# jamie8johnson/cqs

Measured on AMD Instinct MI355X. Metric: queries/sec @k=20 (brute-force cosine scan + top-k, 768-d fp32), higher is better.
Workload: dtype f32; 1 GPU; BASELINE configs[1]: 1000000 x 768 fp32 unit vectors, 1 query per step, brute-force cosine top-20; mode=single, rows_per_gpu=1000000, total_rows=1000000, dim=768, k=20, parallelism=single GPU, ranks_seen=1

## Files before the change

cqs_amd/csrc/index.hip:

```cpp
#include <hip/hip_runtime.h>

#include <algorithm>
#include <atomic>
#include <cmath>
#include <cerrno>
#include <chrono>
#include <cstdio>
#include <cstdlib>
#include <cstring>
#include <mutex>
#include <new>
#include <string>
#include <thread>
#include <vector>

#include <fcntl.h>
#include <libgen.h>
#include <sys/stat.h>
#include <unistd.h>

#include "abi_guard.h"
#include "roctx.h"
#include "index_internal.h"
#include "persist_util.h"
// ... 1 lines not shown
#include "scan_i8.h"

using cqs::kMaxK;
using cqs::kRowsPerBlock;

namespace cqs_idx {

uint64_t pad_rows(uint64_t n) { return (n + kRowsPerBlock - 1) / kRowsPerBlock * kRowsPerBlock; }

int32_t fail(cqs_hip_index* idx, int32_t code, const char* what, hipError_t e) {
    char buf[512];
    if (e != hipSuccess)
        snprintf(buf, sizeof buf, "%s: %s (%s)", what, hipGetErrorString(e), hipGetErrorName(e));
    else
        snprintf(buf, sizeof buf, "%s", what);
    if (idx) {
        idx->last_error = buf;
        if (code == CQS_HIP_ERR_DEVICE) idx->poisoned.store(true, std::memory_order_release);
    }
    return code;
}

void free_scratch(cqs_hip_index* x) {
    hipFree(x->d_q); hipFree(x->d_scores); hipFree(x->d_gmax); hipFree(x->d_work); hipFree(x->d_gaux);
    x->d_work = nullptr; x->d_gaux = nullptr;
    hipFree(x->d_out_keys); hipFree(x->d_out_counts);
    hipHostFree(x->h_q); hipHostFree(x->h_out_keys); hipHostFree(x->h_out_counts);
    x->d_q = x->d_scores = nullptr; x->d_gmax = nullptr;
    x->d_out_keys = nullptr; x->d_out_counts = nullptr;
    x->h_q = nullptr; x->h_out_keys = nullptr; x->h_out_counts = nullptr;
    x->h_out_keys_dev = nullptr; x->h_out_counts_dev = nullptr;
    x->q_cap = 0; x->k_cap = 0; x->scr_n_pad = 0;
}

int32_t ensure_scratch(cqs_hip_index* x, uint32_t b, uint32_t k) {
    const uint64_t n_pad = pad_rows(x->n);
    if (b <= x->q_cap && k <= x->k_cap && n_pad == x->scr_n_pad) return CQS_HIP_OK;
    HIP_TRY(x, hipDeviceSynchronize());
    uint32_t qc = x->q_cap > b ? x->q_cap : b;
    uint32_t kc = x->k_cap > k ? x->k_cap : k;
    free_scratch(x);
    HIP_TRY(x, hipMalloc(&x->d_q, ((size_t)qc + 256) * x->dim * sizeof(float)));
    HIP_TRY(x, hipMalloc(&x->d_scores, (size_t)qc * n_pad * sizeof(float)));
    HIP_TRY(x, hipMalloc(&x->d_work, cqs::kWorkWords * sizeof(uint32_t)));
    HIP_TRY(x, hipMemset(x->d_work, 0, cqs::kWorkWords * sizeof(uint32_t)));
    HIP_TRY(x, hipMalloc(&x->d_gmax, (size_t)qc * (n_pad / cqs::kTaskRowsSmall) * sizeof(float)));
    HIP_TRY(x, hipMalloc(&x->d_gaux, (size_t)(qc < kGauxQueries ? qc : kGauxQueries) * (n_pad / cqs::kTaskRowsSmall) * sizeof(uint64_t)));
    HIP_TRY(x, hipMalloc(&x->d_out_keys, (size_t)qc * kc * sizeof(uint64_t)));
    HIP_TRY(x, hipMalloc(&x->d_out_counts, (size_t)qc * sizeof(uint32_t)));
    HIP_TRY(x, hipHostMalloc(&x->h_q, (size_t)qc * x->dim * sizeof(float), hipHostMallocDefault));
    HIP_TRY(x, hipHostMalloc(&x->h_out_keys, (size_t)qc * kc * sizeof(uint64_t), hipHostMallocDefault));
    HIP_TRY(x, hipHostMalloc(&x->h_out_counts, (size_t)qc * sizeof(uint32_t), hipHostMallocDefault));
    if (hipHostGetDevicePointer((void**)&x->h_out_keys_dev, x->h_out_keys, 0) != hipSuccess ||
        hipHostGetDevicePointer((void**)&x->h_out_counts_dev, x->h_out_counts, 0) != hipSuccess) {
        (void)hipGetLastError();
        x->h_out_keys_dev = nullptr; x->h_out_counts_dev = nullptr;
    }
    x->q_cap = qc; x->k_cap = kc; x->scr_n_pad = n_pad;
    return CQS_HIP_OK;
}

uint32_t max_query_block(const cqs_hip_index* x) {
    const uint64_t budget = 16ull << 30;
    const uint64_t per_q = pad_rows(x->n) * sizeof(float);
    uint64_t q = per_q ? budget / per_q : 1024;
    if (q < 1) q = 1;
    if (q > 1024) q = 1024;
    return (uint32_t)q;
}

// ... 1043 lines not shown
```

cqs_amd/csrc/index_internal.h:

```cpp
#pragma once
#include <hip/hip_runtime.h>

#include <atomic>
#include <chrono>
#include <condition_variable>
#include <deque>
#include <mutex>
#include <string>
#include <vector>

#include "../../include/cqs_hip.h"
#include "scan_kernels.h"

namespace cqs_sharded { struct ShardSet; }
namespace cqs_idx { struct Shadow; }
namespace cqs_mmr { struct Scratch; }

struct cqs_combine_req {
    const float* q;
    uint32_t k, mode;
    float thr;
    uint64_t* out_rows;
    float* out_scores;
    uint32_t* out_count;
// ... 3 lines not shown
};

struct cqs_hip_index {
    int device = 0;
    uint64_t n = 0;
    uint64_t cap_rows = 0;
    uint32_t dim = 0;
    uint32_t metric = 0;
    uint64_t row_base = 0;
    bool borrow = false;
    float* d_rows = nullptr;
    hipStream_t stream = nullptr;

    uint32_t q_cap = 0;
    uint64_t scr_n_pad = 0;
    uint32_t k_cap = 0;
    float* d_q = nullptr;
    float* d_scores = nullptr;
    uint32_t* d_work = nullptr;
    unsigned long long* d_dbg = nullptr;
    uint32_t n_cu = 256;
    float* d_gmax = nullptr;
    uint64_t* d_gaux = nullptr;
    uint64_t* d_out_keys = nullptr;
    uint32_t* d_out_counts = nullptr;
    uint32_t* d_keep = nullptr;
    uint64_t keep_words_cap = 0;
    uint32_t* d_keep_tab = nullptr;
    uint32_t* h_keep_tab = nullptr;
    uint64_t keep_tab_stride = 0;
    float* h_q = nullptr;
    uint64_t* h_out_keys = nullptr;
    uint32_t* h_out_counts = nullptr;
    uint64_t* h_out_keys_dev = nullptr;
    uint32_t* h_out_counts_dev = nullptr;

    hipEvent_t done = nullptr;
    hipStream_t done_stream = nullptr;
    bool done_valid = false;

    bool timing = false;
    std::vector<hipEvent_t> ev;
    size_t ev_used = 0;

    cqs_sharded::ShardSet* sh = nullptr;

// ... 121 lines not shown
```

cqs_amd/csrc/index_shadow.hip:

```cpp
#include <cstdlib>
#include <cstring>
#include <new>

#include "abi_guard.h"
#include "index_internal.h"
#include "scan_bf16.h"
#include "scan_i8.h"

namespace cqs_idx {

constexpr uint64_t kShadowAutoBytes = 1ull << 30;
constexpr uint64_t kShadowFreeMinBytes = 4ull << 30;
constexpr double kShadowFreeFrac = 0.10;
constexpr uint32_t kStatWords = 10, kStatCounts = 3, kStatI8 = 5, kStatI8Counts = 8;

struct Shadow {
    uint16_t* d_bf16 = nullptr;
    uint64_t cap = 0;
    int8_t* d_i8 = nullptr;
    float* d_i8_scale = nullptr;
    double r8 = 0.0, norm8 = 0.0;
    double r = 0.0;
    double norm = 0.0;
    unsigned long long* d_stats = nullptr;
// ... 235 lines not shown
bool shadow_takes(const cqs_hip_index* x, uint32_t b, uint32_t k, bool gemv_only) {
    return x->shadow && b <= cqs::kShadowMaxQ && (gemv_only || !cqs::use_mfma(b, x->dim)) && cqs::shadow_kprime(k) >= k;
}

bool shadow_uses_i8(const cqs_hip_index* x, uint32_t b, uint32_t k) {
    return x->shadow && x->shadow->d_i8 && b <= cqs::kI8MaxQ && cqs::i8_k_ok(k);
}

int32_t shadow_pass(cqs_hip_index* x, const float* d_q, uint32_t nb, uint32_t k, const uint32_t* d_keep, uint32_t mode,
                    float threshold, uint64_t* out_keys, uint32_t* out_counts, hipStream_t st, const uint32_t** device_gate,
                    const KeepTab* tab) {
    const Shadow* s = x->shadow;
    uint32_t* const cert = device_gate || !s->h_cert_dev ? s->d_cert : s->h_cert_dev;
    if (device_gate) *device_gate = cert;
    if (device_gate) HIP_TRY(x, order_after_last(x, st));
    const bool i8 = shadow_uses_i8(x, nb, k);
    const uint32_t kp = i8 ? cqs::i8_kprime(k) : cqs::shadow_kprime(k);
    const double r_max = i8 ? s->r8 : s->r, norm_max = i8 ? s->norm8 : s->norm;
    const bool bound_first = mode == CQS_HIP_MODE_PIPELINE;
    if (bound_first) {
        if (i8) HIP_TRY(x, cqs::launch_i8_bound(d_q, nb, x->dim, r_max, norm_max, s->d_bq, st));
        else HIP_TRY(x, cqs::launch_shadow_bound(d_q, nb, x->dim, r_max, norm_max, s->d_bq, st));
    }
    const cqs::ScanArgs a = scan_args(x, d_q, nb, kp + 1u, d_keep, mode, threshold, i8 ? sizeof(int8_t) : sizeof(uint16_t), true, nullptr, nullptr, tab);
    const ShadowRows rows{i8 ? nullptr : s->d_bf16, i8 ? s->d_i8 : nullptr, s->d_i8_scale, s->d_bq};
    const int32_t rc = scan_select(x, a, st, &rows, nullptr, nullptr);
    if (rc == CQS_HIP_OK)
        HIP_TRY(x, cqs::launch_rescore_certify(a, (uint32_t)x->row_base, k, kp, bound_first ? 0u : (i8 ? 2u : 1u), r_max, norm_max,
                                               s->d_bq, s->d_tickets, s->d_ekeys, out_keys, out_counts, cert,
                                               device_gate ? s->d_stats + kStatCounts : nullptr,
                                               device_gate && i8 ? s->d_stats + kStatI8Counts : nullptr, st));
    return rc;
}

hipError_t shadow_verdicts(cqs_hip_index* x, uint32_t nb, const uint32_t** h_cert) {
    const Shadow* s = x->shadow;
    *h_cert = s->h_cert;
    return s->h_cert_dev ? hipSuccess : hipMemcpyAsync(s->h_cert, s->d_cert, (size_t)nb * sizeof(uint32_t), hipMemcpyDeviceToHost, x->stream);
}

}

using namespace cqs_idx;

extern "C" {

int32_t cqs_hip_index_set_bf16_scan(cqs_hip_index* x, int32_t enable) CQS_ABI_TRY {
// ... 148 lines not shown
        if ((rc = stage_keep(x, keep_bitset, (x->n + 31) / 32)) != CQS_HIP_OK) return rc;
        d_keep = x->d_keep;
    }
    hipStream_t st = x->stream;
    HIP_TRY(x, hipMemcpyAsync(x->d_q, queries, (size_t)b * x->dim * sizeof(float), hipMemcpyHostToDevice, st));
    if (i8) HIP_TRY(x, cqs::launch_i8_bound(x->d_q, b, x->dim, s->r8, s->norm8, s->d_bq, st));
    else HIP_TRY(x, cqs::launch_shadow_bound(x->d_q, b, x->dim, s->r, s->norm, s->d_bq, st));
    if (copy == 0u) {
        const cqs::ScanArgs a = scan_args(x, x->d_q, b, k, d_keep, mode, threshold, sizeof(float), false, x->d_dbg, nullptr);
        HIP_TRY(x, cqs::launch_scan(a, st));
    } else {
        const cqs::ScanArgs a = scan_args(x, x->d_q, b, k_scan, d_keep, mode, threshold, i8 ? sizeof(int8_t) : sizeof(uint16_t), true, nullptr, nullptr);
        if (i8) HIP_TRY(x, cqs::launch_scan_i8(a, s->d_i8, s->d_i8_scale, s->d_bq, st));
        else HIP_TRY(x, cqs::launch_scan_bf16(a, s->d_bf16, s->d_bq, st));
    }
    HIP_TRY(x, hipMemsetAsync(x->d_work, 0, cqs::kWorkWords * sizeof(uint32_t), st));
    const size_t row_b = (size_t)x->n * sizeof(float);
    HIP_TRY(x, hipMemcpy2DAsync(out_scores, row_b, x->d_scores, (size_t)pad_rows(x->n) * sizeof(float), row_b, b, hipMemcpyDeviceToHost, st));
    HIP_TRY(x, hipMemcpyAsync(out_bq, s->d_bq, (size_t)b * sizeof(float), hipMemcpyDeviceToHost, st));
    HIP_TRY(x, hipStreamSynchronize(st));
    return CQS_HIP_OK;
} CQS_ABI_CATCH(x)

}
```

cqs_amd/csrc/scan_bf16.hip:

```cpp
#include "scan_bf16.h"
#include "scan_i8.h"
#include "launch_util.h"
#include "rank_sort.h"
#include "scan_gemv_device.h"
#include "select_device.h"

namespace cqs {

static_assert(kShadowKMax == kMaxK, "shadow k' policy and the select agree on max k");

typedef __bf16 bf2 __attribute__((ext_vector_type(2)));

__device__ __forceinline__ float bf_lo(uint32_t w) { return __uint_as_float(w << 16); }
__device__ __forceinline__ float bf_hi(uint32_t w) { return __uint_as_float(w & 0xFFFF0000u); }
__device__ __forceinline__ float key_score(uint64_t key) {
    const uint32_t ok = (uint32_t)(key >> 32);
    return __uint_as_float((ok & 0x80000000u) ? (ok ^ 0x80000000u) : ~ok);
}

__global__ __launch_bounds__(256) void shadow_build_kernel(const float* __restrict__ rows, uint16_t* __restrict__ shadow,
                                                           uint64_t row0, uint64_t n_rows, uint32_t dim, double gamma,
                                                           unsigned long long* __restrict__ stats) {
    const int lane = threadIdx.x & 63;
    const uint64_t waves = (uint64_t)gridDim.x * (blockDim.x >> 6);
// ... 288 lines not shown
}

hipError_t launch_scan_bf16(const ScanArgs& a, const uint16_t* shadow, const float* bq, hipStream_t st) {
    if (a.b == 0 || a.n == 0) return hipSuccess;
    if (a.b > kShadowMaxQ || a.dim % 8u != 0u || a.dim > kShadowMaxDim) return hipErrorInvalidValue;
    if (a.keep_tab && !keep_tab_ok(a)) return hipErrorInvalidValue;
    switch ((a.dim + 511u) / 512u) {
        case 1: return a.keep_tab ? launch_bf16_groups<1, true>(a, shadow, bq, st) : launch_bf16_groups<1, false>(a, shadow, bq, st);
        case 2: return a.keep_tab ? launch_bf16_groups<2, true>(a, shadow, bq, st) : launch_bf16_groups<2, false>(a, shadow, bq, st);
        case 3: return a.keep_tab ? launch_bf16_groups<3, true>(a, shadow, bq, st) : launch_bf16_groups<3, false>(a, shadow, bq, st);
        case 4: return a.keep_tab ? launch_bf16_groups<4, true>(a, shadow, bq, st) : launch_bf16_groups<4, false>(a, shadow, bq, st);
        default: return hipErrorInvalidValue;
    }
}

struct TailParams {
    const float* rows;
    const float* q;
    uint32_t dim, k, kprime, mode, row_base;
    float thr;
    const float* scores;
    const float* gmax;
    const uint64_t* gaux;
    uint32_t n_pad;
    TaskTiers tiers;
    uint32_t bins;
    uint32_t* work;
    uint64_t* ekeys;
    float* bq;
    uint32_t* tickets;
    uint32_t bound;
    double r_max, norm_max;
    uint64_t* out_keys;
    uint32_t* out_counts;
    uint32_t* cert;
    unsigned long long* counters;
    unsigned long long* counters2;
};

constexpr uint32_t kTailWaves = 16;

template <int NCH>
__global__ __launch_bounds__(1024) void rescore_certify_kernel(const TailParams p) {
    __shared__ uint64_t s_keys[kShadowKMax];
    __shared__ uint64_t s_sorted[kShadowKMax];
    __shared__ __attribute__((aligned(16))) uint32_t s_ok[kShadowKMax + 4];
    __shared__ uint32_t s_cnt, s_flag, s_last;
    const uint32_t lane = threadIdx.x & 63u;
    const uint32_t qi = blockIdx.y;
    const uint32_t wave = (uint32_t)__builtin_amdgcn_readfirstlane((int)(blockIdx.x * kTailWaves + (threadIdx.x >> 6)));
    const uint32_t n_waves = gridDim.x * kTailWaves;
    const uint32_t dim = p.dim;
    const float* qp = p.q + (size_t)qi * dim;
    if (threadIdx.x == 0) s_cnt = 0u;
    if (qi == 0u && blockIdx.x == 0u)
        for (uint32_t i = threadIdx.x; i < kWorkWords; i += 1024u) p.work[i] = 0u;

    const uint32_t n_tasks = p.tiers.total();
    uint32_t found;
    const uint64_t* akeys = select_body(p.scores + (size_t)qi * p.n_pad, p.gmax + (size_t)qi * n_tasks,
                                        p.gaux ? p.gaux + (size_t)qi * n_tasks : nullptr, p.n_pad, p.tiers, p.kprime + 1u,
                                        p.row_base, p.bins, nullptr, found);
    const uint32_t ac = found < p.kprime + 1u ? found : p.kprime + 1u;
    const uint32_t nc = ac < p.kprime ? ac : p.kprime;
    const uint64_t key_next = ac > p.kprime ? akeys[p.kprime] : 0ull;

    for (uint32_t slot = wave; slot <= nc; slot += n_waves) {
        if (slot == 0u) {
            if (p.bound != 0u) {
                const float v = p.bound == 2u ? wave_i8_bound(qp, dim, p.r_max, p.norm_max, lane)
                                              : wave_shadow_bound(qp, dim, p.r_max, p.norm_max, lane);
                if (lane == 0u)
                    __hip_atomic_store((uint32_t*)p.bq + qi, __float_as_uint(v), __ATOMIC_RELAXED, __HIP_MEMORY_SCOPE_AGENT);
            }
            continue;
        }
        const uint32_t i = slot - 1u;
        const uint64_t key = akeys[i];
        const uint32_t grow = 0xFFFFFFFFu - (uint32_t)key;
        const float* rp = p.rows + (size_t)(grow - p.row_base) * dim;
        f4 x[NCH], qv[NCH];
#pragma unroll
        for (int c = 0; c < NCH; ++c) {
            const uint32_t idx = (uint32_t)c * 256u + lane * 4u;
            const bool in = idx < dim;
// ... 54 lines not shown
                if (p.mode == 1u) t = t < 0.f ? 0.f : (t > 1.f ? 1.f : t);
                ok = t < key_score(s_sorted[k - 1u]);
            }
        }
        p.cert[qi] = ok ? 1u : 0u;
        if (p.counters) atomicAdd(&p.counters[ok ? 0 : 1], 1ull);
        if (p.counters2) atomicAdd(&p.counters2[ok ? 0 : 1], 1ull);
    }
}

#ifndef CQS_TAIL_MAX_BLOCKS_PER_CU
#define CQS_TAIL_MAX_BLOCKS_PER_CU 1u
#endif

hipError_t launch_rescore_certify(const ScanArgs& a, uint32_t row_base, uint32_t k, uint32_t kprime, uint32_t bound,
                                  double r_max, double norm_max, float* bq, uint32_t* tickets, uint64_t* ekeys,
                                  uint64_t* out_keys, uint32_t* out_counts, uint32_t* cert, unsigned long long* counters,
                                  unsigned long long* counters2, hipStream_t st) {
    const uint32_t b = a.b, dim = a.dim;
    if (b == 0) return hipSuccess;
    if (b > kShadowMaxQ || k == 0 || kprime < k || kprime >= kShadowKMax || a.k != kprime + 1u || dim % 8u != 0u ||
        dim > kShadowMaxDim || bound > 2u)
        return hipErrorInvalidValue;
    const TailParams tp{a.rows, a.q, dim, k, kprime, a.mode, row_base, a.threshold, a.scores, a.gmax, a.gaux, a.n_pad, a.tiers,
                        a.range_bins ? 2u : (a.linear_bins ? 1u : 0u), a.work, ekeys, bq, tickets, bound, r_max, norm_max,
                        out_keys, out_counts, cert, counters, counters2};
    const uint32_t want = (kprime + 1u + kTailWaves - 1u) / kTailWaves;
    uint32_t cap = a.n_cu * CQS_TAIL_MAX_BLOCKS_PER_CU / b;
    if (cap < 1u) cap = 1u;
    const dim3 grid(want < cap ? want : cap, b), block(64u * kTailWaves);
    switch ((dim + 255u) / 256u) {
        case 1: hipLaunchKernelGGL(rescore_certify_kernel<1>, grid, block, 0, st, tp); break;
        case 2: hipLaunchKernelGGL(rescore_certify_kernel<2>, grid, block, 0, st, tp); break;
        case 3: hipLaunchKernelGGL(rescore_certify_kernel<3>, grid, block, 0, st, tp); break;
        case 4: hipLaunchKernelGGL(rescore_certify_kernel<4>, grid, block, 0, st, tp); break;
        case 5: hipLaunchKernelGGL(rescore_certify_kernel<5>, grid, block, 0, st, tp); break;
        case 6: hipLaunchKernelGGL(rescore_certify_kernel<6>, grid, block, 0, st, tp); break;
        case 7: hipLaunchKernelGGL(rescore_certify_kernel<7>, grid, block, 0, st, tp); break;
        case 8: hipLaunchKernelGGL(rescore_certify_kernel<8>, grid, block, 0, st, tp); break;
        default: return hipErrorInvalidValue;
    }
    return hipGetLastError();
}

}
```

cqs_amd/csrc/scan_i8.hip:

```cpp
#include "scan_i8.h"
#include "launch_util.h"
#include "scan_gemv_device.h"

namespace cqs {

template <int I>
__device__ __forceinline__ float code_f32(uint32_t w) { return (float)(int)(int8_t)(w >> (8 * I)); }

constexpr int kI8BuildVecs = (int)(kShadowMaxDim / 256u);

__global__ __launch_bounds__(256) void i8_build_kernel(const float* __restrict__ rows, int8_t* __restrict__ codes,
                                                       float* __restrict__ scales, uint64_t row0, uint64_t n_rows,
                                                       uint32_t dim, double gamma, unsigned long long* __restrict__ stats) {
    const uint32_t lane = threadIdx.x & 63u;
    const uint64_t waves = (uint64_t)gridDim.x * (blockDim.x >> 6);
    for (uint64_t r = (uint64_t)blockIdx.x * (blockDim.x >> 6) + (threadIdx.x >> 6); r < n_rows; r += waves) {
        const float* xp = rows + (row0 + r) * dim;
        int8_t* op = codes + (row0 + r) * dim;
        f4 v[kI8BuildVecs];
        float m = 0.f;
        bool fin = true;
#pragma unroll
        for (int j = 0; j < kI8BuildVecs; ++j) {
            const uint32_t i = (uint32_t)j * 256u + lane * 4u;
// ... 48 lines not shown
hipError_t launch_i8_build(const float* rows, int8_t* codes, float* scales, uint64_t row0, uint64_t n_rows, uint32_t dim,
                           double gamma, unsigned long long* stats, hipStream_t st) {
    if (n_rows == 0) return hipSuccess;
    if (!i8_dim_ok(dim)) return hipErrorInvalidValue;
    const uint64_t blocks = (n_rows + 3u) / 4u;
    hipLaunchKernelGGL(i8_build_kernel, dim3((uint32_t)(blocks < 8192u ? blocks : 8192u)), dim3(256), 0, st, rows, codes,
                       scales, row0, n_rows, dim, gamma, stats);
    return hipGetLastError();
}

__global__ __launch_bounds__(64) void i8_bound_kernel(const float* __restrict__ q, uint32_t dim, double r_max,
                                                      double norm_max, float* __restrict__ bq) {
    const uint32_t lane = threadIdx.x;
    const float v = wave_i8_bound(q + (size_t)blockIdx.x * dim, dim, r_max, norm_max, lane);
    if (lane == 0) bq[blockIdx.x] = v;
}

hipError_t launch_i8_bound(const float* q, uint32_t b, uint32_t dim, double r_max, double norm_max, float* bq, hipStream_t st) {
    if (b == 0) return hipSuccess;
    if (b > kShadowMaxQ) return hipErrorInvalidValue;
    hipLaunchKernelGGL(i8_bound_kernel, dim3(b), dim3(64), 0, st, q, dim, r_max, norm_max, bq);
    return hipGetLastError();
}

struct I8ScanParams {
    const int8_t* rows;
    const float* scales;
    uint32_t n, n_pad, dim;
    const float* q;
    float* scores;
    const uint32_t* keep;
    uint32_t mode;
    float thr;
    uint32_t nq;
    TaskTiers tiers;
    uint32_t n_tasks;
    float* gmax;
    uint64_t* gaux;
    const float* bq;
    uint32_t keep_stride;
    uint8_t slot[kMaxGemvQ];
};

template <int NCH, int BQ, int RI, bool NT, bool FULL, bool PQ>
__global__ __launch_bounds__(256) void scan_i8_kernel(const I8ScanParams p) {
    constexpr int NV = RI * BQ;
    constexpr int LPV = 64 / NV;
    const int lane = threadIdx.x & 63;
    const uint32_t n = p.n, dim = p.dim;

    uint32_t coff[NCH];
    f4 qv[BQ][NCH][4];
#pragma unroll
    for (int c = 0; c < NCH; ++c) {
        const uint32_t idx = (uint32_t)c * 1024u + (uint32_t)lane * 16u;
        const bool in = FULL || idx < dim;
        coff[c] = in ? idx : dim - 16u;
#pragma unroll
        for (int b = 0; b < BQ; ++b) {
            const float* qp = p.q + (size_t)((uint32_t)b < p.nq ? b : 0) * dim + coff[c];
#pragma unroll
            for (int w = 0; w < 4; ++w) {
                const f4 t = *(const f4*)(qp + 4 * w);
                qv[b][c][w] = in ? t : (f4)(0.f);
            }
        }
    }

    const uint32_t last = n - 1u;
    const uint32_t nwords = (n + 31u) / 32u;
    const uint32_t n_tasks = p.n_tasks;
    const uint32_t wpb = blockDim.x >> 6;
// ... 45 lines not shown
        for (int b = 0; b < BQ; ++b) {
            const float t = __shfl(acc[0], (b * RI + (lane % RI)) * LPV, 64);
            if (lane / RI == j) sc[b] = t;
        }
    };
    uint64_t qmask[PQ ? BQ : 1];
    auto epilogue = [&](uint32_t cur, uint32_t base, uint32_t trows, uint64_t mask, float scale, float (&sc)[BQ]) {
        const uint32_t row = base + (uint32_t)lane;
        const bool live_all = (uint32_t)lane < trows && ((mask >> lane) & 1ull);
#pragma unroll
        for (int b = 0; b < BQ; ++b) {
            const bool live = PQ ? (uint32_t)lane < trows && ((qmask[PQ ? b : 0] >> lane) & 1ull) : live_all;
            float s = sc[b] * scale;
            if (!live || !(__builtin_fabsf(s) <= 3.4028234664e38f)) s = -INFINITY;
            else if (p.mode == 1u && (uint32_t)b < p.nq) {
                float t = s + p.bq[b];
                t = t < 0.f ? 0.f : (t > 1.f ? 1.f : t);
                if (!(t >= p.thr)) s = -INFINITY;
            }
            if ((uint32_t)b >= p.nq) continue;
            if ((uint32_t)lane < trows && row < p.n_pad) p.scores[(size_t)b * p.n_pad + row] = s;
            const float gm = wave_max64(s);
            if (lane == 0) p.gmax[(size_t)b * n_tasks + cur] = gm;
            if (p.gaux) {
                const uint32_t arg = (uint32_t)__builtin_ctzll(__ballot(s == gm));
                const float sec = wave_max64(((uint32_t)lane == arg) ? -INFINITY : s);
                if (lane == 0) p.gaux[(size_t)b * n_tasks + cur] = ((uint64_t)arg << 32) | (uint64_t)__float_as_uint(sec);
            }
        }
    };
    auto task_mask = [&](uint32_t base, uint32_t trows) -> uint64_t {
        const uint64_t all = trows == 64u ? ~0ull : ((1ull << trows) - 1ull);
        uint64_t mask = all;
        if (base + trows > n) mask = (base >= n) ? 0ull : (all >> (trows - (n - base)));
        if constexpr (PQ) {
            const uint32_t w = base / 32u;
            uint64_t any = 0ull;
#pragma unroll
            for (int b = 0; b < BQ; ++b) {
                uint64_t m = 0ull;
                if ((uint32_t)b < p.nq) {
                    const kc32* kp = (const kc32*)(p.keep + (size_t)p.slot[b] * p.keep_stride);
                    const uint32_t w0 = (w < nwords) ? kp[w] : 0u;
                    const uint32_t w1 = (w + 1u < nwords) ? kp[w + 1u] : 0u;
                    m = mask & ((((uint64_t)w1 << 32) | (uint64_t)w0) >> (base & 31u));
                }
                const uint32_t mlo = __builtin_amdgcn_readfirstlane((uint32_t)m);
                const uint32_t mhi = __builtin_amdgcn_readfirstlane((uint32_t)(m >> 32));
                qmask[b] = ((uint64_t)mhi << 32) | mlo;
                any |= qmask[b];
// ... 19 lines not shown
    const float scale = p.scales[srow > last ? last : srow];
    float sc[BQ];
#pragma unroll
    for (int b = 0; b < BQ; ++b) sc[b] = -INFINITY;
    const int nb = (int)(trows / (uint32_t)RI);
    for (int j = 0; j < nb; ++j) {
        const uint32_t m = (uint32_t)(mask >> (RI * j)) & ((1u << RI) - 1u);
        if (m == 0u) continue;
        load_rows(base, j, x);
        reduce_rows(j, x, sc);
    }
    epilogue(cur, base, trows, mask, scale, sc);
}

constexpr int kI8RowsPerBatch = 16;

template <int NCH, int BQ, int RI, bool PQ>
static hipError_t launch_i8(const ScanArgs& a, const int8_t* codes, const float* scales, const float* bq, uint32_t q0,
                            uint32_t nq, hipStream_t st) {
    I8ScanParams p;
    fill_gemv_pass(p, a, q0, nq, PQ);
    p.rows = codes; p.scales = scales;
    p.bq = bq + q0;
    const uint32_t wpb = 4u;
    const dim3 grid((p.n_tasks + wpb - 1u) / wpb), block(64u * wpb);
    const bool full = (a.dim == (uint32_t)NCH * 1024u);
    for_nt_full(a.nontemporal, full, [&](auto nt_c, auto full_c) {
        hipLaunchKernelGGL((scan_i8_kernel<NCH, BQ, RI, decltype(nt_c)::value, decltype(full_c)::value, PQ>), grid, block, 0, st, p);
    });
    return hipGetLastError();
}

template <int NCH, bool PQ>
static hipError_t launch_i8_groups(const ScanArgs& a, const int8_t* codes, const float* scales, const float* bq, hipStream_t st) {
    uint32_t done = 0;
    while (done < a.b) {
        const uint32_t left = a.b - done;
        hipError_t e;
        uint32_t g;
        if (left >= 3) { g = left < 4u ? left : 4u; e = launch_i8<NCH, 4, 4, PQ>(a, codes, scales, bq, done, g, st); }
        else if (left >= 2) { g = 2; e = launch_i8<NCH, 2, 8, PQ>(a, codes, scales, bq, done, g, st); }
        else { g = 1; e = launch_i8<NCH, 1, kI8RowsPerBatch, PQ>(a, codes, scales, bq, done, g, st); }
        if (e != hipSuccess) return e;
        done += g;
    }
    return hipSuccess;
}
// ... 14 lines not shown
```

cqs_amd/csrc/scan_kernels.h:

```cpp
#pragma once
#include <hip/hip_runtime.h>
#include <stdint.h>

namespace cqs {

constexpr uint32_t kTaskRows = 64;
constexpr uint32_t kTaskRowsSmall = 16;
constexpr uint32_t kRowsPerBlock = 256;
constexpr uint32_t kHistBins = 4096;
constexpr uint32_t kCandCap = 8192;
constexpr uint32_t kMaxK = 1024;
constexpr uint32_t kMaxGemvQ = 8;
constexpr uint32_t kDbgWaves = 4096;
constexpr uint32_t kWorkWords = 64;

struct TaskTiers {
    uint32_t nA, nB, nC;
    __host__ __device__ uint32_t total() const { return nA + nB + nC; }
    __host__ __device__ uint32_t locate(uint32_t t, uint32_t& rows) const {
        if (t < nA) { rows = 64u; return t * 64u; }
        if (t < nA + nB) { rows = 32u; return nA * 64u + (t - nA) * 32u; }
        rows = 16u;
        return nA * 64u + nB * 32u + (t - nA - nB) * 16u;
    }
};
TaskTiers plan_tiers(uint32_t n_pad, uint32_t n_cu, bool uniform64);

struct ScanArgs {
    const float* rows;
    uint32_t n;
    uint32_t n_pad;
    uint32_t dim;
    const float* q;
    uint32_t b;
    float* scores;
    const uint32_t* keep;
    const uint32_t* keep_tab = nullptr;
    uint32_t keep_stride = 0;
    const uint8_t* keep_slot = nullptr;
    uint32_t mode;
    float threshold;
    bool nontemporal;
    bool linear_bins;
    bool range_bins = false;
    uint32_t k;
    float* gmax;
    uint64_t* gaux = nullptr;
    TaskTiers tiers;
    uint32_t* work;
    uint32_t n_cu;
    bool gemv_only = false;
    void* dbg;
    const uint32_t* gate = nullptr;
};

hipError_t launch_scan(const ScanArgs& a, hipStream_t stream);

hipError_t launch_select(const ScanArgs& a, uint32_t row_base, uint64_t* out_keys, uint32_t* out_counts,
                         hipStream_t stream);

hipError_t launch_scan_mfma(const ScanArgs& a, uint32_t q0, uint32_t nq, uint32_t work_slot, hipStream_t stream);
uint32_t mfma_query_tile(uint32_t nq);
constexpr uint32_t kMfmaMinQueries = 9;
inline bool use_mfma(uint32_t b, uint32_t dim) { return b >= kMfmaMinQueries && dim % 32u == 0; }
inline bool uniform_groups(uint32_t b, uint32_t dim) { return use_mfma(b, dim); }

bool scan_dim_supported(uint32_t dim);

inline bool keep_tab_ok(const ScanArgs& a) {
    return !a.keep && a.keep_slot && a.keep_stride >= (a.n + 31u) / 32u;
// ... 32 lines not shown
```

cqs_amd/csrc/scan_kernels.hip:

```cpp
#include "scan_kernels.h"
#include "launch_util.h"
#include "scan_gemv_device.h"
#include "select_device.h"

namespace cqs {


struct ScanParams {
    const float* rows;
    uint32_t n, n_pad, dim;
    const float* q;
    float* scores;
    const uint32_t* keep;
    uint32_t mode;
    float thr;
    uint32_t nq;
    uint32_t* work;
    TaskTiers tiers;
    uint32_t n_tasks;
    float* gmax;
    uint64_t* gaux;
    unsigned long long* dbg;
    const uint32_t* gate;
    uint32_t gate_n;
// ... 183 lines not shown
            if (use_queue && lane == 0) ticket = atomicAdd(p.work + zero, 1u);
            sparse_task(cur, base, trows, mask);
        }
        cur = claimed(ticket);
    }
    if (p.dbg && lane == 0 && wave_id < kDbgWaves) p.dbg[17u + 2u * wave_id] = __builtin_amdgcn_s_memrealtime();
}

__global__ __launch_bounds__(1024) void select_finish_kernel(const float* __restrict__ scores,
                                                             const float* __restrict__ gmax,
                                                             const uint64_t* __restrict__ gaux, uint32_t n_pad,
                                                             const TaskTiers tiers, uint32_t slot_log2, uint32_t k,
                                                             uint32_t row_base, uint32_t linear,
                                                             uint64_t* __restrict__ out_keys,
                                                             uint32_t* __restrict__ out_counts,
                                                             uint32_t* __restrict__ work,
                                                             unsigned long long* __restrict__ dbg,
                                                             const uint32_t* __restrict__ gate, uint32_t gate_n) {
    if (gate && gate_closed(gate, gate_n)) return;
    const uint32_t qi = blockIdx.x;
    const uint32_t n_tasks = tiers.total();
    uint32_t count;
    const uint64_t* sorted = select_body(scores + (size_t)qi * n_pad, gmax + (size_t)qi * n_tasks,
                                         gaux ? gaux + (size_t)qi * n_tasks : nullptr, n_pad, tiers, k, row_base, linear, dbg,
                                         count);
    const uint32_t outc = count < k ? count : k;
    for (uint32_t i = threadIdx.x; i < k; i += 1024u) out_keys[(size_t)qi * k + i] = (i < outc) ? sorted[i] : 0ull;
    if (threadIdx.x == 0) out_counts[qi] = outc;
    if (qi == 0) for (uint32_t i = threadIdx.x; i < kWorkWords; i += 1024u) work[i] = 0u;
    if (dbg && threadIdx.x == 0 && blockIdx.x == 0) dbg[6] = __builtin_amdgcn_s_memrealtime();
}

bool scan_dim_supported(uint32_t dim) { return dim >= 4 && dim % 4 == 0 && dim <= 4096; }

#ifndef CQS_SCAN_PIPE
#define CQS_SCAN_PIPE 1
#endif
#ifndef CQS_SCAN_RI1
#define CQS_SCAN_RI1 8
#endif
#ifndef CQS_SCAN_CAP_OCCUPANCY
#define CQS_SCAN_CAP_OCCUPANCY 1
#endif
#ifndef CQS_SCAN_ONE_SHOT
#define CQS_SCAN_ONE_SHOT 24u
#endif
#ifndef CQS_SCAN_BLOCK_WAVES
// ... 160 lines not shown
```

cqs_amd/csrc/select_device.h:

```cpp
#pragma once
#include <hip/hip_runtime.h>
#include <stdint.h>

#include "rank_sort.h"
#include "scan_device.h"
#include "scan_kernels.h"

namespace cqs {

__device__ __forceinline__ uint32_t bin_of(float s, bool linear) {
    if (linear) {
        const float t = (s + 1.0f) * 2048.0f;
        const int b = (int)t;
        return (uint32_t)(b < 0 ? 0 : (b > 4095 ? 4095 : b));
    }
    return okey(s) >> 20;
}
__device__ __forceinline__ uint32_t bin_of_range(float s, float lo, float scale) {
    if (!(scale > 0.f)) return 0u;
    const float t = (s - lo) * scale;
    if (!(t < 4095.0f)) return 4095u;
    return t > 0.f ? (uint32_t)(int)t : 0u;
}
__device__ __forceinline__ uint32_t bin_any(float s, uint32_t mode, float lo, float scale) {
    return mode == 2u ? bin_of_range(s, lo, scale) : bin_of(s, mode != 0u);
// ... 72 lines not shown
        sel_above += above;
        k_rem -= above;
        lb = prefix << (64 - bits_done);
        if (sel_above + cnt <= kCandCap) break;
    }
    if (threadIdx.x == 0) *s_cnt = 0;
    __syncthreads();
    for (uint32_t i = threadIdx.x; i < n_pad; i += 1024u) {
        const uint32_t kk = okey(s[i]);
        if (kk <= kInvalidKey) continue;
        const uint64_t key = pack_key(kk, row_base + i);
        if (key >= lb) {
            const uint32_t slot = atomicAdd(s_cnt, 1u);
            if (slot < kCandCap) s_keys[slot] = key;
        }
    }
    __syncthreads();
    const uint32_t c = *s_cnt;
    return c < kCandCap ? c : kCandCap;
}

constexpr uint32_t kGroupCap = 8192;
constexpr int kGB = 16;

__device__ __forceinline__ const uint64_t* select_body(const float* __restrict__ s, const float* __restrict__ gm,
                                                       const uint64_t* __restrict__ ga, uint32_t n_pad,
                                                       const TaskTiers& tiers, uint32_t k, uint32_t row_base,
                                                       uint32_t linear, unsigned long long* __restrict__ dbg,
                                                       uint32_t& count_out) {
    __shared__ uint64_t s_keys[kCandCap];
    __shared__ uint32_t s_groups[kGroupCap];
    __shared__ __attribute__((aligned(16))) uint32_t s_hist[kHistBins];
    __shared__ uint32_t s_part[1024];
    __shared__ uint32_t s_res[4];
    __shared__ uint32_t s_cnt, s_ng, s_ng2;
    const uint32_t n_tasks = tiers.total();
    const int lane = threadIdx.x & 63;
    float r_lo = 0.f, r_scale = 0.f;

#define CQS_STAMP(i) do { if (dbg && threadIdx.x == 0 && blockIdx.x == 0) dbg[i] = __builtin_amdgcn_s_memrealtime(); } while (0)
    CQS_STAMP(0);
    for (uint32_t i = threadIdx.x; i < kHistBins; i += 1024u) s_hist[i] = 0u;
    if (threadIdx.x == 0) { s_cnt = 0; s_ng = 0; s_ng2 = 0; }
    __syncthreads();
    if (linear == 2u) {
        float lo = INFINITY, hi = -INFINITY;
        for (uint32_t t0 = 0; t0 < n_tasks; t0 += 1024u * kGB) {
            float v[kGB];
#pragma unroll
            for (int u = 0; u < kGB; ++u) {
                const uint32_t t = t0 + (uint32_t)u * 1024u + threadIdx.x;
                v[u] = gm[t < n_tasks ? t : n_tasks - 1u];
            }
#pragma unroll
            for (int u = 0; u < kGB; ++u)
                if (v[u] != -INFINITY) { lo = fminf(lo, v[u]); hi = fmaxf(hi, v[u]); }
        }
#pragma unroll
        for (int off = 32; off >= 1; off >>= 1) {
            lo = fminf(lo, __shfl_xor(lo, off, 64));
            hi = fmaxf(hi, __shfl_xor(hi, off, 64));
        }
        float* const f_part = reinterpret_cast<float*>(s_part);
        if (lane == 0) { f_part[threadIdx.x >> 6] = lo; f_part[16 + (threadIdx.x >> 6)] = hi; }
        __syncthreads();
        lo = f_part[0]; hi = f_part[16];
        for (int w = 1; w < 16; ++w) { lo = fminf(lo, f_part[w]); hi = fmaxf(hi, f_part[16 + w]); }
        __syncthreads();
        r_lo = lo;
        r_scale = (hi > lo) ? 4096.0f / (hi - lo) : 0.f;
        if (!(r_scale < INFINITY)) r_scale = 0.f;
    }

    float m[kGB];
    const bool one_pass = n_tasks <= 1024u * kGB;
    for (uint32_t t0 = 0; t0 < n_tasks; t0 += 1024u * kGB) {
#pragma unroll
        for (int u = 0; u < kGB; ++u) {
            const uint32_t t = t0 + (uint32_t)u * 1024u + threadIdx.x;
            const float v = gm[t < n_tasks ? t : n_tasks - 1u];
            m[u] = t < n_tasks ? v : -INFINITY;
        }
#pragma unroll
        for (int u = 0; u < kGB; ++u)
            if (m[u] != -INFINITY) atomicAdd(&s_hist[bin_any(m[u], linear, r_lo, r_scale)], 1u);
    }
    __syncthreads();
    CQS_STAMP(1);
    block_decide<1024>(s_hist, k, s_part, s_res);
    const uint32_t T = (s_res[3] < k) ? 0u : s_res[0];
    __syncthreads();
    CQS_STAMP(2);

    for (uint32_t t0 = 0; t0 < n_tasks; t0 += 1024u * kGB) {
        if (!one_pass) {
#pragma unroll
            for (int u = 0; u < kGB; ++u) {
                const uint32_t t = t0 + (uint32_t)u * 1024u + threadIdx.x;
                const float v = gm[t < n_tasks ? t : n_tasks - 1u];
                m[u] = t < n_tasks ? v : -INFINITY;
            }
        }
        bool take[kGB];
        uint64_t mk[kGB];
        uint32_t pre[kGB], tot = 0;
#pragma unroll
        for (int u = 0; u < kGB; ++u) {
            take[u] = (m[u] != -INFINITY) && (bin_any(m[u], linear, r_lo, r_scale) >= T);
            mk[u] = __ballot(take[u]);
            pre[u] = tot;
            tot += (uint32_t)__popcll(mk[u]);
        }
        uint32_t base = 0;
        if (tot) {
            if (lane == 0) base = atomicAdd(&s_ng, tot);
            base = (uint32_t)__builtin_amdgcn_readfirstlane((int)base);
        }
#pragma unroll
        for (int u = 0; u < kGB; ++u) {
            const uint32_t slot = base + pre[u] + __builtin_amdgcn_mbcnt_hi((uint32_t)(mk[u] >> 32), __builtin_amdgcn_mbcnt_lo((uint32_t)mk[u], 0u));
            if (take[u] && slot < kGroupCap) s_groups[slot] = t0 + (uint32_t)u * 1024u + threadIdx.x;
        }
    }
    __syncthreads();
    CQS_STAMP(3);
    const uint32_t ng = s_ng;
    uint32_t count = kCandCap + 1u;
    if (ng <= kGroupCap) {
        const uint32_t* glist = s_groups;
        uint32_t n2 = ng;
        if (ga) {
            uint32_t* const s_list2 = s_hist;
            for (uint32_t i0 = 0; i0 < ng; i0 += 1024u) {
                const uint32_t i = i0 + threadIdx.x;
                const bool valid = i < ng;
                const uint32_t t = s_groups[valid ? i : ng - 1u];
                const uint64_t ax = ga[t];
                const float mx = gm[t];
                const float sec = __uint_as_float((uint32_t)ax);
                const bool need = valid && (sec != -INFINITY) && (bin_any(sec, linear, r_lo, r_scale) >= T);
                const bool direct = valid && !need;
                const uint64_t mn = __ballot(need), md = __ballot(direct);
                uint32_t bn = 0, bd = 0;
                if (lane == 0) {
// ... 106 lines not shown
```

Measured before the change: 6595 queries/s.

## Add per-workgroup second-level maxima to i8 scan for hierarchical select

The int8 shadow scan kernel now also reduces the per-wave task maxima within each 4-wave workgroup and writes a coarser gmax2 array. The select stage builds its threshold histogram over these coarse maxima and only expands the surviving workgroups back to per-task maxima. This cuts the histogram and filter passes over the per-task array, which has roughly n/64 entries per query. In exchange it adds shared-memory arrival counting in the scan kernel, an extra scratch buffer and a second filtering stage, and the coarser threshold may let more groups through. A debug entry point for dumping both maxima levels is also added.

```diff
diff --git a/cqs_amd/csrc/index.hip b/cqs_amd/csrc/index.hip
--- a/cqs_amd/csrc/index.hip
+++ b/cqs_amd/csrc/index.hip
@@ -47,8 +47,8 @@
 }
 
 void free_scratch(cqs_hip_index* x) {
-    hipFree(x->d_q); hipFree(x->d_scores); hipFree(x->d_gmax); hipFree(x->d_work); hipFree(x->d_gaux);
-    x->d_work = nullptr; x->d_gaux = nullptr;
+    hipFree(x->d_q); hipFree(x->d_scores); hipFree(x->d_gmax); hipFree(x->d_work); hipFree(x->d_gaux); hipFree(x->d_gmax2);
+    x->d_work = nullptr; x->d_gaux = nullptr; x->d_gmax2 = nullptr;
     hipFree(x->d_out_keys); hipFree(x->d_out_counts);
     hipHostFree(x->h_q); hipHostFree(x->h_out_keys); hipHostFree(x->h_out_counts);
     x->d_q = x->d_scores = nullptr; x->d_gmax = nullptr;
@@ -71,6 +71,7 @@
     HIP_TRY(x, hipMemset(x->d_work, 0, cqs::kWorkWords * sizeof(uint32_t)));
     HIP_TRY(x, hipMalloc(&x->d_gmax, (size_t)qc * (n_pad / cqs::kTaskRowsSmall) * sizeof(float)));
     HIP_TRY(x, hipMalloc(&x->d_gaux, (size_t)(qc < kGauxQueries ? qc : kGauxQueries) * (n_pad / cqs::kTaskRowsSmall) * sizeof(uint64_t)));
+    HIP_TRY(x, hipMalloc(&x->d_gmax2, (size_t)(qc < cqs::kShadowMaxQ ? qc : cqs::kShadowMaxQ) * ((n_pad / cqs::kTaskRowsSmall + 3u) / 4u) * sizeof(float)));
     HIP_TRY(x, hipMalloc(&x->d_out_keys, (size_t)qc * kc * sizeof(uint64_t)));
     HIP_TRY(x, hipMalloc(&x->d_out_counts, (size_t)qc * sizeof(uint32_t)));
     HIP_TRY(x, hipHostMalloc(&x->h_q, (size_t)qc * x->dim * sizeof(float), hipHostMallocDefault));
diff --git a/cqs_amd/csrc/index_internal.h b/cqs_amd/csrc/index_internal.h
--- a/cqs_amd/csrc/index_internal.h
+++ b/cqs_amd/csrc/index_internal.h
@@ -49,6 +49,7 @@
     uint32_t n_cu = 256;
     float* d_gmax = nullptr;
     uint64_t* d_gaux = nullptr;
+    float* d_gmax2 = nullptr;
     uint64_t* d_out_keys = nullptr;
     uint32_t* d_out_counts = nullptr;
     uint32_t* d_keep = nullptr;
diff --git a/cqs_amd/csrc/index_shadow.hip b/cqs_amd/csrc/index_shadow.hip
--- a/cqs_amd/csrc/index_shadow.hip
+++ b/cqs_amd/csrc/index_shadow.hip
@@ -281,7 +281,8 @@
         if (i8) HIP_TRY(x, cqs::launch_i8_bound(d_q, nb, x->dim, r_max, norm_max, s->d_bq, st));
         else HIP_TRY(x, cqs::launch_shadow_bound(d_q, nb, x->dim, r_max, norm_max, s->d_bq, st));
     }
-    const cqs::ScanArgs a = scan_args(x, d_q, nb, kp + 1u, d_keep, mode, threshold, i8 ? sizeof(int8_t) : sizeof(uint16_t), true, nullptr, nullptr, tab);
+    cqs::ScanArgs a = scan_args(x, d_q, nb, kp + 1u, d_keep, mode, threshold, i8 ? sizeof(int8_t) : sizeof(uint16_t), true, nullptr, nullptr, tab);
+    if (i8) a.gmax2 = x->d_gmax2;
     const ShadowRows rows{i8 ? nullptr : s->d_bf16, i8 ? s->d_i8 : nullptr, s->d_i8_scale, s->d_bq};
     const int32_t rc = scan_select(x, a, st, &rows, nullptr, nullptr);
     if (rc == CQS_HIP_OK)
@@ -476,4 +477,52 @@
     return CQS_HIP_OK;
 } CQS_ABI_CATCH(x)
 
-}
+int32_t cqs_hip_debug_i8_maxima(cqs_hip_index* x, const float* queries, uint32_t b, uint32_t k, const uint32_t* keep_bitsets,
+                                uint32_t keep_rows, uint32_t mode, float threshold, float* out_gmax, float* out_gmax2,
+                                uint64_t cap_words, uint32_t* out_n_tasks) CQS_ABI_TRY {
+    if (!x || x->sh || !queries || !out_gmax || !out_gmax2 || !out_n_tasks || b == 0 || mode > CQS_HIP_MODE_PIPELINE) return CQS_HIP_ERR_INVALID;
+    if (k == 0 || k > cqs::kMaxK || (keep_bitsets ? (keep_rows != 1u && keep_rows != b) : keep_rows != 0u)) return CQS_HIP_ERR_INVALID;
+    std::lock_guard<std::mutex> g(x->mu);
+    if (x->poisoned.load(std::memory_order_acquire)) return CQS_HIP_ERR_POISONED;
+    const Shadow* s = x->shadow;
+    if (!s || x->n == 0 || !s->d_i8 || b > cqs::kI8MaxQ || !cqs::i8_k_ok(k) || !shadow_takes(x, b, k, false)) return CQS_HIP_ERR_INVALID;
+    HIP_TRY(x, hipSetDevice(x->device));
+    HIP_TRY(x, quiesce(x));
+    const uint32_t k_scan = cqs::i8_kprime(k) + 1u;
+    int32_t rc = ensure_scratch(x, b, k_scan);
+    if (rc != CQS_HIP_OK) return rc;
+    hipStream_t st = x->stream;
+    const uint64_t words = (x->n + 31) / 32;
+    const uint32_t* d_keep = nullptr;
+    uint8_t slot[cqs::kI8MaxQ];
+    KeepTab tab{nullptr, 0u, slot};
+    const bool per_query = keep_bitsets && keep_rows == b && b > 1u;
+    if (per_query) {
+        if (!ensure_keep_tab(x)) return fail(x, CQS_HIP_ERR_NOMEM, "debug_i8_maxima: no bitset table");
+        for (uint32_t i = 0; i < b; ++i) {
+            memcpy(x->h_keep_tab + i * x->keep_tab_stride, keep_bitsets + i * words, words * sizeof(uint32_t));
+            slot[i] = (uint8_t)i;
+        }
+        HIP_TRY(x, hipMemcpyAsync(x->d_keep_tab, x->h_keep_tab, ((size_t)(b - 1u) * x->keep_tab_stride + words) * sizeof(uint32_t),
+                                  hipMemcpyHostToDevice, st));
+        tab.d_tab = x->d_keep_tab; tab.stride = (uint32_t)x->keep_tab_stride;
+    } else if (keep_bitsets) {
+        if ((rc = stage_keep(x, keep_bitsets, words)) != CQS_HIP_OK) return rc;
+        d_keep = x->d_keep;
+    }
+    HIP_TRY(x, hipMemcpyAsync(x->d_q, queries, (size_t)b * x->dim * sizeof(float), hipMemcpyHostToDevice, st));
+    HIP_TRY(x, cqs::launch_i8_bound(x->d_q, b, x->dim, s->r8, s->norm8, s->d_bq, st));
+    cqs::ScanArgs a = scan_args(x, x->d_q, b, k_scan, d_keep, mode, threshold, sizeof(int8_t), true, nullptr, nullptr, per_query ? &tab : nullptr);
+    a.gmax2 = x->d_gmax2;
+    const uint32_t n_tasks = a.tiers.total(), n_wg = (n_tasks + 3u) / 4u;
+    if ((uint64_t)b * n_tasks > cap_words) return CQS_HIP_ERR_INVALID;
+    HIP_TRY(x, cqs::launch_scan_i8(a, s->d_i8, s->d_i8_scale, s->d_bq, st));
+    HIP_TRY(x, hipMemsetAsync(x->d_work, 0, cqs::kWorkWords * sizeof(uint32_t), st));
+    HIP_TRY(x, hipMemcpyAsync(out_gmax, x->d_gmax, (size_t)b * n_tasks * sizeof(float), hipMemcpyDeviceToHost, st));
+    HIP_TRY(x, hipMemcpyAsync(out_gmax2, x->d_gmax2, (size_t)b * n_wg * sizeof(float), hipMemcpyDeviceToHost, st));
+    HIP_TRY(x, hipStreamSynchronize(st));
+    *out_n_tasks = n_tasks;
+    return CQS_HIP_OK;
+} CQS_ABI_CATCH(x)
+
+}
diff --git a/cqs_amd/csrc/scan_bf16.hip b/cqs_amd/csrc/scan_bf16.hip
--- a/cqs_amd/csrc/scan_bf16.hip
+++ b/cqs_amd/csrc/scan_bf16.hip
@@ -334,6 +334,7 @@
     const float* scores;
     const float* gmax;
     const uint64_t* gaux;
+    const float* gmax2;
     uint32_t n_pad;
     TaskTiers tiers;
     uint32_t bins;
@@ -371,8 +372,9 @@
     const uint32_t n_tasks = p.tiers.total();
     uint32_t found;
     const uint64_t* akeys = select_body(p.scores + (size_t)qi * p.n_pad, p.gmax + (size_t)qi * n_tasks,
-                                        p.gaux ? p.gaux + (size_t)qi * n_tasks : nullptr, p.n_pad, p.tiers, p.kprime + 1u,
-                                        p.row_base, p.bins, nullptr, found);
+                                        p.gaux ? p.gaux + (size_t)qi * n_tasks : nullptr,
+                                        p.gmax2 ? p.gmax2 + (size_t)qi * ((n_tasks + 3u) / 4u) : nullptr, p.n_pad, p.tiers,
+                                        p.kprime + 1u, p.row_base, p.bins, nullptr, found);
     const uint32_t ac = found < p.kprime + 1u ? found : p.kprime + 1u;
     const uint32_t nc = ac < p.kprime ? ac : p.kprime;
     const uint64_t key_next = ac > p.kprime ? akeys[p.kprime] : 0ull;
@@ -473,7 +475,7 @@
     if (b > kShadowMaxQ || k == 0 || kprime < k || kprime >= kShadowKMax || a.k != kprime + 1u || dim % 8u != 0u ||
         dim > kShadowMaxDim || bound > 2u)
         return hipErrorInvalidValue;
-    const TailParams tp{a.rows, a.q, dim, k, kprime, a.mode, row_base, a.threshold, a.scores, a.gmax, a.gaux, a.n_pad, a.tiers,
+    const TailParams tp{a.rows, a.q, dim, k, kprime, a.mode, row_base, a.threshold, a.scores, a.gmax, a.gaux, a.gmax2, a.n_pad, a.tiers,
                         a.range_bins ? 2u : (a.linear_bins ? 1u : 0u), a.work, ekeys, bq, tickets, bound, r_max, norm_max,
                         out_keys, out_counts, cert, counters, counters2};
     const uint32_t want = (kprime + 1u + kTailWaves - 1u) / kTailWaves;
diff --git a/cqs_amd/csrc/scan_i8.hip b/cqs_amd/csrc/scan_i8.hip
--- a/cqs_amd/csrc/scan_i8.hip
+++ b/cqs_amd/csrc/scan_i8.hip
@@ -94,6 +94,8 @@
     hipLaunchKernelGGL(i8_bound_kernel, dim3(b), dim3(64), 0, st, q, dim, r_max, norm_max, bq);
     return hipGetLastError();
 }
+
+constexpr uint32_t kI8BlockWaves = 4;
 
 struct I8ScanParams {
     const int8_t* rows;
@@ -109,6 +111,7 @@
     uint32_t n_tasks;
     float* gmax;
     uint64_t* gaux;
+    float* gmax2;
     const float* bq;
     uint32_t keep_stride;
     uint8_t slot[kMaxGemvQ];
@@ -120,6 +123,10 @@
     constexpr int LPV = 64 / NV;
     const int lane = threadIdx.x & 63;
     const uint32_t n = p.n, dim = p.dim;
+    __shared__ float s_gm[BQ][kI8BlockWaves];
+    __shared__ uint32_t s_arrived;
+    if (threadIdx.x == 0) s_arrived = 0u;
+    __syncthreads();
 
     uint32_t coff[NCH];
     f4 qv[BQ][NCH][4];
@@ -211,10 +218,28 @@
             if ((uint32_t)lane < trows && row < p.n_pad) p.scores[(size_t)b * p.n_pad + row] = s;
             const float gm = wave_max64(s);
             if (lane == 0) p.gmax[(size_t)b * n_tasks + cur] = gm;
+            if (p.gmax2 && lane == 0) s_gm[b][threadIdx.x >> 6] = gm;
             if (p.gaux) {
                 const uint32_t arg = (uint32_t)__builtin_ctzll(__ballot(s == gm));
                 const float sec = wave_max64(((uint32_t)lane == arg) ? -INFINITY : s);
                 if (lane == 0) p.gaux[(size_t)b * n_tasks + cur] = ((uint64_t)arg << 32) | (uint64_t)__float_as_uint(sec);
+            }
+        }
+        if (p.gmax2) {
+            __atomic_signal_fence(__ATOMIC_SEQ_CST);
+            uint32_t t = 0u;
+            if (lane == 0) t = __hip_atomic_fetch_add(&s_arrived, 1u, __ATOMIC_RELAXED, __HIP_MEMORY_SCOPE_WORKGROUP);
+            t = (uint32_t)__builtin_amdgcn_readfirstlane((int)t);
+            __atomic_signal_fence(__ATOMIC_SEQ_CST);
+            const uint32_t left = n_tasks - blockIdx.x * kI8BlockWaves;
+            const uint32_t live = left < kI8BlockWaves ? left : kI8BlockWaves;
+            if (t == live - 1u && (uint32_t)lane < p.nq && lane < BQ) {
+                const float* g = s_gm[lane];
+                float m = g[0];
+#pragma unroll
+                for (uint32_t w = 1; w < kI8BlockWaves; ++w)
+                    if (w < live) m = fmaxf(m, g[w]);
+                p.gmax2[(size_t)lane * gridDim.x + blockIdx.x] = m;
             }
         }
     };
@@ -280,7 +305,8 @@
     fill_gemv_pass(p, a, q0, nq, PQ);
     p.rows = codes; p.scales = scales;
     p.bq = bq + q0;
-    const uint32_t wpb = 4u;
+    const uint32_t wpb = kI8BlockWaves;
+    p.gmax2 = a.gmax2 ? a.gmax2 + (size_t)q0 * ((p.n_tasks + wpb - 1u) / wpb) : nullptr;
     const dim3 grid((p.n_tasks + wpb - 1u) / wpb), block(64u * wpb);
     const bool full = (a.dim == (uint32_t)NCH * 1024u);
     for_nt_full(a.nontemporal, full, [&](auto nt_c, auto full_c) {
diff --git a/cqs_amd/csrc/scan_kernels.h b/cqs_amd/csrc/scan_kernels.h
--- a/cqs_amd/csrc/scan_kernels.h
+++ b/cqs_amd/csrc/scan_kernels.h
@@ -46,6 +46,7 @@
     uint32_t k;
     float* gmax;
     uint64_t* gaux = nullptr;
+    float* gmax2 = nullptr;
     TaskTiers tiers;
     uint32_t* work;
     uint32_t n_cu;
diff --git a/cqs_amd/csrc/scan_kernels.hip b/cqs_amd/csrc/scan_kernels.hip
--- a/cqs_amd/csrc/scan_kernels.hip
+++ b/cqs_amd/csrc/scan_kernels.hip
@@ -229,7 +229,7 @@
     const uint32_t n_tasks = tiers.total();
     uint32_t count;
     const uint64_t* sorted = select_body(scores + (size_t)qi * n_pad, gmax + (size_t)qi * n_tasks,
-                                         gaux ? gaux + (size_t)qi * n_tasks : nullptr, n_pad, tiers, k, row_base, linear, dbg,
+                                         gaux ? gaux + (size_t)qi * n_tasks : nullptr, nullptr, n_pad, tiers, k, row_base, linear, dbg,
                                          count);
     const uint32_t outc = count < k ? count : k;
     for (uint32_t i = threadIdx.x; i < k; i += 1024u) out_keys[(size_t)qi * k + i] = (i < outc) ? sorted[i] : 0ull;
diff --git a/cqs_amd/csrc/select_device.h b/cqs_amd/csrc/select_device.h
--- a/cqs_amd/csrc/select_device.h
+++ b/cqs_amd/csrc/select_device.h
@@ -1,6 +1,8 @@
 #pragma once
 #include <hip/hip_runtime.h>
 #include <stdint.h>
+
+#include <type_traits>
 
 #include "rank_sort.h"
 #include "scan_device.h"
@@ -119,9 +121,12 @@
 
 constexpr uint32_t kGroupCap = 8192;
 constexpr int kGB = 16;
+constexpr uint32_t kWgCap = 8192;
+constexpr int kWB = 4;
 
 __device__ __forceinline__ const uint64_t* select_body(const float* __restrict__ s, const float* __restrict__ gm,
-                                                       const uint64_t* __restrict__ ga, uint32_t n_pad,
+                                                       const uint64_t* __restrict__ ga, const float* __restrict__ gm2,
+                                                       uint32_t n_pad,
                                                        const TaskTiers& tiers, uint32_t k, uint32_t row_base,
                                                        uint32_t linear, unsigned long long* __restrict__ dbg,
                                                        uint32_t& count_out) {
@@ -130,7 +135,7 @@
     __shared__ __attribute__((aligned(16))) uint32_t s_hist[kHistBins];
     __shared__ uint32_t s_part[1024];
     __shared__ uint32_t s_res[4];
-    __shared__ uint32_t s_cnt, s_ng, s_ng2;
+    __shared__ uint32_t s_cnt, s_ng, s_ng2, s_nw;
     const uint32_t n_tasks = tiers.total();
     const int lane = threadIdx.x & 63;
     float r_lo = 0.f, r_scale = 0.f;
@@ -138,7 +143,7 @@
 #define CQS_STAMP(i) do { if (dbg && threadIdx.x == 0 && blockIdx.x == 0) dbg[i] = __builtin_amdgcn_s_memrealtime(); } while (0)
     CQS_STAMP(0);
     for (uint32_t i = threadIdx.x; i < kHistBins; i += 1024u) s_hist[i] = 0u;
-    if (threadIdx.x == 0) { s_cnt = 0; s_ng = 0; s_ng2 = 0; }
+    if (threadIdx.x == 0) { s_cnt = 0; s_ng = 0; s_ng2 = 0; s_nw = 0; }
     __syncthreads();
     if (linear == 2u) {
         float lo = INFINITY, hi = -INFINITY;
@@ -169,54 +174,159 @@
         if (!(r_scale < INFINITY)) r_scale = 0.f;
     }
 
-    float m[kGB];
-    const bool one_pass = n_tasks <= 1024u * kGB;
-    for (uint32_t t0 = 0; t0 < n_tasks; t0 += 1024u * kGB) {
-#pragma unroll
-        for (int u = 0; u < kGB; ++u) {
-            const uint32_t t = t0 + (uint32_t)u * 1024u + threadIdx.x;
-            const float v = gm[t < n_tasks ? t : n_tasks - 1u];
-            m[u] = t < n_tasks ? v : -INFINITY;
-        }
-#pragma unroll
-        for (int u = 0; u < kGB; ++u)
-            if (m[u] != -INFINITY) atomicAdd(&s_hist[bin_any(m[u], linear, r_lo, r_scale)], 1u);
-    }
-    __syncthreads();
-    CQS_STAMP(1);
-    block_decide<1024>(s_hist, k, s_part, s_res);
-    const uint32_t T = (s_res[3] < k) ? 0u : s_res[0];
-    __syncthreads();
-    CQS_STAMP(2);
-
-    for (uint32_t t0 = 0; t0 < n_tasks; t0 += 1024u * kGB) {
-        if (!one_pass) {
+    uint32_t T;
+    if (gm2) {
+        const uint32_t n_wg = (n_tasks + 3u) >> 2;
+        float m[kGB];
+        auto load_trip = [&](uint32_t t0) {
+            auto load_n = [&](auto gb) {
+#pragma unroll
+                for (int u = 0; u < kGB; ++u) {
+                    if (u < decltype(gb)::value) {
+                        const uint32_t t = t0 + (uint32_t)u * 1024u + threadIdx.x;
+                        const float v = gm2[t < n_wg ? t : n_wg - 1u];
+                        m[u] = t < n_wg ? v : -INFINITY;
+                    } else {
+                        m[u] = -INFINITY;
+                    }
+                }
+            };
+            if (n_wg - t0 <= 4u * 1024u) load_n(std::integral_constant<int, 4>{});
+            else load_n(std::integral_constant<int, kGB>{});
+        };
+        const bool one_pass = n_wg <= 1024u * kGB;
+        for (uint32_t t0 = 0; t0 < n_wg; t0 += 1024u * kGB) {
+            load_trip(t0);
+#pragma unroll
+            for (int u = 0; u < kGB; ++u)
+                if (m[u] != -INFINITY) atomicAdd(&s_hist[bin_any(m[u], linear, r_lo, r_scale)], 1u);
+        }
+        __syncthreads();
+        CQS_STAMP(1);
+        block_decide<1024>(s_hist, k, s_part, s_res);
+        T = (s_res[3] < k) ? 0u : s_res[0];
+        __syncthreads();
+        CQS_STAMP(2);
+
+        uint32_t* const s_wlist = reinterpret_cast<uint32_t*>(s_keys);
+        for (uint32_t t0 = 0; t0 < n_wg; t0 += 1024u * kGB) {
+            if (!one_pass) load_trip(t0);
+            bool take[kGB];
+            uint64_t mk[kGB];
+            uint32_t pre[kGB], tot = 0;
+#pragma unroll
+            for (int u = 0; u < kGB; ++u) {
+                take[u] = (m[u] != -INFINITY) && (bin_any(m[u], linear, r_lo, r_scale) >= T);
+                mk[u] = __ballot(take[u]);
+                pre[u] = tot;
+                tot += (uint32_t)__popcll(mk[u]);
+            }
+            uint32_t base = 0;
+            if (tot) {
+                if (lane == 0) base = atomicAdd(&s_nw, tot);
+                base = (uint32_t)__builtin_amdgcn_readfirstlane((int)base);
+            }
+#pragma unroll
+            for (int u = 0; u < kGB; ++u) {
+                const uint32_t slot = base + pre[u] + __builtin_amdgcn_mbcnt_hi((uint32_t)(mk[u] >> 32), __builtin_amdgcn_mbcnt_lo((uint32_t)mk[u], 0u));
+                if (take[u] && slot < kWgCap) s_wlist[slot] = t0 + (uint32_t)u * 1024u + threadIdx.x;
+            }
+        }
+        __syncthreads();
+        const uint32_t nw = s_nw;
+        if (nw > kWgCap) {
+            if (threadIdx.x == 0) s_ng = kGroupCap + 1u;
+        } else {
+            const uint32_t ne = nw * 4u;
+            auto list_trip = [&](uint32_t i0, auto wb) {
+                constexpr int WB = decltype(wb)::value;
+                float v[WB];
+                uint32_t tt[WB];
+#pragma unroll
+                for (int u = 0; u < WB; ++u) {
+                    const uint32_t i = i0 + (uint32_t)u * 1024u + threadIdx.x;
+                    const uint32_t t = s_wlist[i < ne ? i >> 2 : 0u] * 4u + (i & 3u);
+                    const bool in = i < ne && t < n_tasks;
+                    tt[u] = t;
+                    const float g = gm[in ? t : n_tasks - 1u];
+                    v[u] = in ? g : -INFINITY;
+                }
+                bool take[WB];
+                uint64_t mk[WB];
+                uint32_t pre[WB], tot = 0;
+#pragma unroll
+                for (int u = 0; u < WB; ++u) {
+                    take[u] = (v[u] != -INFINITY) && (bin_any(v[u], linear, r_lo, r_scale) >= T);
+                    mk[u] = __ballot(take[u]);
+                    pre[u] = tot;
+                    tot += (uint32_t)__popcll(mk[u]);
+                }
+                uint32_t base = 0;
+                if (tot) {
+                    if (lane == 0) base = atomicAdd(&s_ng, tot);
+                    base = (uint32_t)__builtin_amdgcn_readfirstlane((int)base);
+                }
+#pragma unroll
+                for (int u = 0; u < WB; ++u) {
+                    const uint32_t slot = base + pre[u] + __builtin_amdgcn_mbcnt_hi((uint32_t)(mk[u] >> 32), __builtin_amdgcn_mbcnt_lo((uint32_t)mk[u], 0u));
+                    if (take[u] && slot < kGroupCap) s_groups[slot] = tt[u];
+                }
+            };
+            for (uint32_t i0 = 0; i0 < ne; i0 += 1024u * kWB) {
+                if (ne - i0 <= 1024u) list_trip(i0, std::integral_constant<int, 1>{});
+                else list_trip(i0, std::integral_constant<int, kWB>{});
+            }
+        }
+    } else {
+        float m[kGB];
+        const bool one_pass = n_tasks <= 1024u * kGB;
+        for (uint32_t t0 = 0; t0 < n_tasks; t0 += 1024u * kGB) {
 #pragma unroll
             for (int u = 0; u < kGB; ++u) {
                 const uint32_t t = t0 + (uint32_t)u * 1024u + threadIdx.x;
                 const float v = gm[t < n_tasks ? t : n_tasks - 1u];
                 m[u] = t < n_tasks ? v : -INFINITY;
             }
-        }
-        bool take[kGB];
-        uint64_t mk[kGB];
-        uint32_t pre[kGB], tot = 0;
-#pragma unroll
-        for (int u = 0; u < kGB; ++u) {
-            take[u] = (m[u] != -INFINITY) && (bin_any(m[u], linear, r_lo, r_scale) >= T);
-            mk[u] = __ballot(take[u]);
-            pre[u] = tot;
-            tot += (uint32_t)__popcll(mk[u]);
-        }
-        uint32_t base = 0;
-        if (tot) {
-            if (lane == 0) base = atomicAdd(&s_ng, tot);
-            base = (uint32_t)__builtin_amdgcn_readfirstlane((int)base);
-        }
-#pragma unroll
-        for (int u = 0; u < kGB; ++u) {
-            const uint32_t slot = base + pre[u] + __builtin_amdgcn_mbcnt_hi((uint32_t)(mk[u] >> 32), __builtin_amdgcn_mbcnt_lo((uint32_t)mk[u], 0u));
-            if (take[u] && slot < kGroupCap) s_groups[slot] = t0 + (uint32_t)u * 1024u + threadIdx.x;
+#pragma unroll
+            for (int u = 0; u < kGB; ++u)
+                if (m[u] != -INFINITY) atomicAdd(&s_hist[bin_any(m[u], linear, r_lo, r_scale)], 1u);
+        }
+        __syncthreads();
+        CQS_STAMP(1);
+        block_decide<1024>(s_hist, k, s_part, s_res);
+        T = (s_res[3] < k) ? 0u : s_res[0];
+        __syncthreads();
+        CQS_STAMP(2);
+
+        for (uint32_t t0 = 0; t0 < n_tasks; t0 += 1024u * kGB) {
+            if (!one_pass) {
+#pragma unroll
+                for (int u = 0; u < kGB; ++u) {
+                    const uint32_t t = t0 + (uint32_t)u * 1024u + threadIdx.x;
+                    const float v = gm[t < n_tasks ? t : n_tasks - 1u];
+                    m[u] = t < n_tasks ? v : -INFINITY;
+                }
+            }
+            bool take[kGB];
+            uint64_t mk[kGB];
+            uint32_t pre[kGB], tot = 0;
+#pragma unroll
+            for (int u = 0; u < kGB; ++u) {
+                take[u] = (m[u] != -INFINITY) && (bin_any(m[u], linear, r_lo, r_scale) >= T);
+                mk[u] = __ballot(take[u]);
+                pre[u] = tot;
+                tot += (uint32_t)__popcll(mk[u]);
+            }
+            uint32_t base = 0;
+            if (tot) {
+                if (lane == 0) base = atomicAdd(&s_ng, tot);
+                base = (uint32_t)__builtin_amdgcn_readfirstlane((int)base);
+            }
+#pragma unroll
+            for (int u = 0; u < kGB; ++u) {
+                const uint32_t slot = base + pre[u] + __builtin_amdgcn_mbcnt_hi((uint32_t)(mk[u] >> 32), __builtin_amdgcn_mbcnt_lo((uint32_t)mk[u], 0u));
+                if (take[u] && slot < kGroupCap) s_groups[slot] = t0 + (uint32_t)u * 1024u + threadIdx.x;
+            }
         }
     }
     __syncthreads();
```

Result: no change. 6558 queries/s (-0.6%).
